# facebookresearch/generative-recommenders

Measured on NVIDIA H100. Metric: user-seqs/sec HSTU-large L=8192 d=256 bf16 fwd+bwd, higher is better.
Workload: dtype bf16

## Files before the change

generative_recommenders_b200/csrc/attn_wgmma_bwd.cu:

```cuda
#include "attn_wgmma_bwd.cuh"

namespace hstu {

template <int D, bool BF16>
__global__ void __launch_bounds__(kAttnThreads, 1) attn_bwd_wgmma_kernel(const __grid_constant__ BwdParams p) {
  bwd_key_tile<D, D, BF16, true>(p);
}

template <int D, bool BF16>
__global__ void __launch_bounds__(kAttnThreads, split_min_blocks(D)) attn_bwd_dkdv_wgmma_kernel(const __grid_constant__ BwdParams p) {
  bwd_key_tile<D, D, BF16, false>(p);
}

template <int D, bool BF16>
__global__ void __launch_bounds__(kAttnThreads, split_min_blocks(D)) attn_bwd_dq_wgmma_kernel(const __grid_constant__ BwdParams p) {
  bwd_dq_body<D, D, BF16>(p);
}

template <bool BF16>
__global__ void dq_convert_kernel(const float* __restrict__ acc, uint16_t* __restrict__ dq, long long rows, int heads, int D,
                                  long long row_stride, long long head_stride, float scale) {
  const long long nvec = rows * heads * (D / 8);
  for (long long idx = (long long)blockIdx.x * blockDim.x + threadIdx.x; idx < nvec; idx += (long long)gridDim.x * blockDim.x) {
    const int v = (int)(idx % (D / 8));
// ... 33 lines not shown
static bool split_dq(const hstu_attn_params& p) {
  return p.dqk == 32 || p.dqk == 256 || p.dqk != p.dv || p.deterministic != 0;
}

static bool fp16_copies(const hstu_attn_params& p) { return p.dtype == HSTU_BF16 && p.dqk == 32 && p.dv == 32; }

size_t wgmma_workspace_bytes(const hstu_attn_params& p, bool bwd) {
  if (!bwd && p.delta_q_len > 0) return wgmma_delta_workspace_bytes(p);
  if (fp16_copies(p)) return fp16_operands_workspace_bytes(p, bwd);
  if (!bwd || split_dq(p)) return 0;
  return (size_t)p.total_rows * p.heads * p.dqk * sizeof(float);
}

template <int D, bool BF16, bool kSplit>
static int launch_bwd_wgmma(const hstu_attn_params& p, cudaStream_t st, const Fp16Operands* f16 = nullptr) {
  if constexpr (kSplit) {
    return launch_bwd_split<D, D, BF16>(p, st, attn_bwd_dkdv_wgmma_kernel<D, BF16>, attn_bwd_dq_wgmma_kernel<D, BF16>, f16);
  } else {
    using Cfg = BwdCfg<D, D, true>;
    const size_t need = wgmma_workspace_bytes(p, true);
    if (p.workspace == nullptr || p.workspace_bytes < need) {
      set_error("hstu_attn_bwd: workspace of %zu bytes required (got %zu)", need, p.workspace_bytes);
      return HSTU_ERR_WORKSPACE;
    }
    const BwdOperands o = bwd_operands(p, f16);
    BwdParams bp = bwd_params(p, f16);
    if (int e = make_tmap_rows_heads(&bp.tmQ, o.src[0], p.total_rows, p.heads, D, o.rs[0], o.hs[0], Cfg::BOX_COLS, Cfg::BQ)) return e;
    if (int e = make_tmap_rows_heads(&bp.tmK, o.src[1], p.total_rows, p.heads, D, o.rs[1], o.hs[1], Cfg::BOX_COLS, Cfg::BKV)) return e;
    if (int e = make_tmap_rows_heads(&bp.tmV, o.src[2], p.total_rows, p.heads, D, o.rs[2], o.hs[2], Cfg::BOX_COLS, Cfg::BKV)) return e;
    if (int e = make_tmap_rows_heads(&bp.tmDO, o.src[3], p.total_rows, p.heads, D, o.rs[3], o.hs[3], Cfg::BOX_COLS, Cfg::BQ)) return e;
    HSTU_CUDA_OK(cudaMemsetAsync(p.workspace, 0, need, st));
    auto kern = attn_bwd_wgmma_kernel<D, BF16>;
    HSTU_CUDA_OK(cudaFuncSetAttribute(kern, cudaFuncAttributeMaxDynamicSharedMemorySize, Cfg::SMEM_BYTES));
    dim3 grid((p.max_seq_len + Cfg::BKV - 1) / Cfg::BKV, p.heads, p.batch);
    kern<<<grid, kAttnThreads, Cfg::SMEM_BYTES, st>>>(bp);
    HSTU_CUDA_OK(cudaGetLastError());
    const long long nvec = p.total_rows * p.heads * (D / 8);
    long long blocks = (nvec + 255) / 256;
    if (blocks > 132 * 16) blocks = 132 * 16;
    dq_convert_kernel<BF16><<<(int)blocks, 256, 0, st>>>(bp.dq_acc, reinterpret_cast<uint16_t*>(p.dq), p.total_rows, p.heads, D,
                                                         p.dq_row_stride, p.dq_head_stride, bp.dk_scale);
    HSTU_CUDA_OK(cudaGetLastError());
    return 0;
  }
}

int attn_wgmma_bwd(const hstu_attn_params& p, cudaStream_t st) {
  if (p.dqk != p.dv) return attn_wgmma_bwd_mixed(p, st);
  const bool bf = p.dtype == HSTU_BF16;
  const bool split = split_dq(p);
  switch (p.dqk) {
    case 32: {
      if (!bf) return launch_bwd_wgmma<32, false, true>(p, st);
      Fp16Operands f16;
      if (int e = fp16_operands_prepass(p, true, &f16, st)) return e;
      return launch_bwd_wgmma<32, false, true>(p, st, &f16);
    }
    case 64:
      if (split) return bf ? launch_bwd_wgmma<64, true, true>(p, st) : launch_bwd_wgmma<64, false, true>(p, st);
      return bf ? launch_bwd_wgmma<64, true, false>(p, st) : launch_bwd_wgmma<64, false, false>(p, st);
    case 128:
      if (split) return bf ? launch_bwd_wgmma<128, true, true>(p, st) : launch_bwd_wgmma<128, false, true>(p, st);
      return bf ? launch_bwd_wgmma<128, true, false>(p, st) : launch_bwd_wgmma<128, false, false>(p, st);
    case 256:
      return bf ? launch_bwd_wgmma<256, true, true>(p, st) : launch_bwd_wgmma<256, false, true>(p, st);
  }
  set_error("wgmma backward: unsupported head dim %d", p.dqk);
// ... 5 lines not shown
```

generative_recommenders_b200/csrc/attn_wgmma_bwd.cuh:

```cuda
#pragma once
#include <string.h>

#include <type_traits>

#include "attn_fp16_operands.cuh"
#include "attn_wgmma_qtile.cuh"
#include "common.cuh"
#include "internal.h"
#include "wgmma.cuh"

namespace hstu {
using namespace wg;

struct alignas(64) BwdParams {
  CUtensorMap tmQ, tmK, tmV, tmDO;
  SeqArgs seq;
  void* dk;
  void* dv;
  float* dq_acc;
  void* dq;
  long long dk_row_stride, dk_head_stride, dv_row_stride, dv_head_stride, dq_row_stride, dq_head_stride;
  float dv_scale;
  float dk_scale;
  const uint32_t* amax;
// ... 34 lines not shown
  static constexpr int K_BYTES = BKV * DQK * 2, V_BYTES = BKV * DV * 2;
  static constexpr int Q_BYTES = BQ * DQK * 2, DO_BYTES = BQ * DV * 2;
  static constexpr int STAGES = DQK != DV ? 4 : DQK == 256 ? 3 : (DQK <= 32 || !FUSED_DQ) ? 4 : (DQK == 64 ? 3 : 2);
  static constexpr int DS_BYTES = BKV * BQ * 2;
  static constexpr int DQN = DQK < 64 ? DQK : 64;
  static constexpr int OFF_K = 0;
  static constexpr int OFF_V = OFF_K + K_BYTES;
  static constexpr int OFF_Q = OFF_V + V_BYTES;
  static constexpr int OFF_DO = OFF_Q + STAGES * Q_BYTES;
  static constexpr int OFF_DS = OFF_DO + STAGES * DO_BYTES;
  static constexpr int OFF_BAR = OFF_DS + (FUSED_DQ ? 4 * DS_BYTES : 0);
  static constexpr int SMEM_BYTES = OFF_BAR + 256 + 1024;
  static_assert(SMEM_BYTES * (FUSED_DQ ? 1 : split_min_blocks(DV)) <= kSmemPerSm, "shared memory budget");
  static_assert(STAGES <= 4, "BwdBars holds four stages");
};

struct BwdBars {
  uint64_t kv_full;
  uint64_t qd_full[4];
  uint32_t qd_free[4];
};

struct QTiles {
  int A, first, T;
  __device__ __forceinline__ int at(int i) const { return i < A ? i : first + (i - A); }
};

template <int DQK, int DV, bool BF16, bool FUSED_DQ>
__device__ __forceinline__ void bwd_key_tile(const BwdParams& p) {
  using Cfg = BwdCfg<DQK, DV, FUSED_DQ>;
  constexpr int SW = Cfg::SW, SWQ = Cfg::SWQ, SWV = Cfg::SWV, BQ = Cfg::BQ, NST = Cfg::STAGES;
  constexpr int NSL = Cfg::NSL, DNK = DQK / NSL, DNV = DV / NSL;
  static_assert(DNK % Cfg::BOX_COLS_Q == 0 && DNV % Cfg::BOX_COLS_V == 0, "a slice is whole boxes");
  const int b = blockIdx.z, h = blockIdx.y;
  const int n0 = (blockIdx.x / NSL) * Cfg::BKV;
  const int ck0 = (blockIdx.x % NSL) * DNK, cv0 = (blockIdx.x % NSL) * DNV;
  const long long row0 = load_index(p.seq.seq_offsets, p.seq.offsets_i64, b);
  int len = (int)(load_index(p.seq.seq_offsets, p.seq.offsets_i64, b + 1) - row0);
  if (len > p.seq.max_seq_len) {
    if (blockIdx.x == 0) {
      zero_rows(p.dk, 2, p.dk_row_stride, (long long)h * p.dk_head_stride, DQK, row0 + p.seq.max_seq_len, row0 + len);
      zero_rows(p.dv, 2, p.dv_row_stride, (long long)h * p.dv_head_stride, DV, row0 + p.seq.max_seq_len, row0 + len);
    }
    len = p.seq.max_seq_len;
  }
  if (n0 >= len) return;
  const int n_tgt = p.seq.num_targets ? (int)load_index(p.seq.num_targets, p.seq.targets_i64, b) : -1;
  const SeqMask msk = make_seq_mask(len, n_tgt, p.seq.win, p.seq.min_full, p.seq.ctx);
  const int nrows = min(Cfg::BKV, len - n0);
  QTiles qt;
  {
    int lo, hi, ctx_hi;
    q_range_for_kv_rows(msk, n0, n0 + nrows, &lo, &hi, &ctx_hi);
    qt.A = (ctx_hi + BQ - 1) / BQ;
    qt.first = max(lo / BQ, qt.A);
    qt.T = qt.A + max(0, (hi + BQ - 1) / BQ - qt.first);
  }

  uint8_t* smem = dyn_smem_1k();
  BwdBars* bars = reinterpret_cast<BwdBars*>(smem + Cfg::OFF_BAR);
  const int tid = threadIdx.x, warp = tid >> 5, lane = tid & 31;
  if (tid == 0) {
    mbar_init(&bars->kv_full, 1);
    for (int i = 0; i < NST; ++i) {
      mbar_init(&bars->qd_full[i], 1);
      bars->qd_free[i] = 0u;
    }
    fence_barrier_init();
  }
  __syncthreads();

  auto load_qd = [&](int j) {
    const int st = j % NST;
// ... 232 lines not shown
        if (kScaled) {
          k0 = scalbnf(k0, sc.e_dk), k1 = scalbnf(k1, sc.e_dk);
          v0 = scalbnf(v0, sc.e_dv), v1 = scalbnf(v1, sc.e_dv);
        }
        const bool out_bf16 = BF16 || p.amax != nullptr;
        if (has_k) *reinterpret_cast<uint32_t*>(krow + nb * 8) = out_bf16 ? pack_bf16x2(k0, k1) : pack_f16x2(k0, k1);
        *reinterpret_cast<uint32_t*>(vrow + nb * 8) = out_bf16 ? pack_bf16x2(v0, v1) : pack_f16x2(v0, v1);
      }
    }
  }
}

template <int DQK, int DV>
struct DqCfg {
  static constexpr int BM = 128;
  static constexpr int BN = DQK + DV >= 384 ? 32 : 64;
  static constexpr int SW = swizzle_bytes(DQK), SWV = swizzle_bytes(DV);
  static constexpr int BOX_COLS = SW / 2, BOX_COLS_V = SWV / 2;
  static constexpr int NBOX = DQK / BOX_COLS, NBOX_V = DV / BOX_COLS_V;
  static constexpr int Q_BOX = BM * SW, DO_BOX = BM * SWV;
  static constexpr int K_BOX = BN * SW, V_BOX = BN * SWV;
  static constexpr int Q_BYTES = BM * DQK * 2, DO_BYTES = BM * DV * 2;
  static constexpr int K_BYTES = BN * DQK * 2, V_BYTES = BN * DV * 2;
  static constexpr int STAGES = 3;
  static constexpr int OFF_Q = 0;
  static constexpr int OFF_DO = OFF_Q + Q_BYTES;
  static constexpr int OFF_K = OFF_DO + DO_BYTES;
  static constexpr int OFF_V = OFF_K + STAGES * K_BYTES;
  static constexpr int OFF_BAR = OFF_V + STAGES * V_BYTES;
  static constexpr int SMEM_BYTES = OFF_BAR + 256 + 1024;
  static_assert(SMEM_BYTES * split_min_blocks(DV) <= kSmemPerSm, "shared memory budget of split_min_blocks(dv) CTAs per SM");
};

template <int DQK, int DV, bool BF16>
__device__ __forceinline__ void bwd_dq_body(const BwdParams& p) {
  using Cfg = DqCfg<DQK, DV>;
  constexpr int SW = Cfg::SW, SWV = Cfg::SWV, BN = Cfg::BN, NST = Cfg::STAGES;
  constexpr bool kScaled = !BF16 && DQK == 32 && DV == 32;
  const int b = blockIdx.z, h = blockIdx.y;
  const int m0 = (int)(gridDim.x - 1 - blockIdx.x) * Cfg::BM;
  QTileSeq qs;
  if (!qtile_prologue<Cfg::BM, BN>(p.seq, b, h, m0, p.dq, p.dq_row_stride, p.dq_head_stride, DQK, &qs)) return;

  uint8_t* smem = dyn_smem_1k();
  KvRing<Cfg> ring{smem, &p.tmK, &p.tmV, h, qs.row0, qs.t0, qs.T};
  ring.init();
  const int tid = threadIdx.x, warp = tid >> 5, lane = tid & 31;
  if (tid == 0) {
    prefetch_tensormap(&p.tmQ);
    prefetch_tensormap(&p.tmK);
    prefetch_tensormap(&p.tmV);
    prefetch_tensormap(&p.tmDO);
    mbar_arrive_expect_tx(&ring.bars->q_full, Cfg::Q_BYTES + Cfg::DO_BYTES);
#pragma unroll
    for (int bx = 0; bx < imax(Cfg::NBOX, Cfg::NBOX_V); ++bx) {
      if (bx < Cfg::NBOX) tma_load_3d(smem + Cfg::OFF_Q + bx * Cfg::Q_BOX, &p.tmQ, &ring.bars->q_full, bx * Cfg::BOX_COLS, h, (int)(qs.row0 + m0));
      if (bx < Cfg::NBOX_V)
        tma_load_3d(smem + Cfg::OFF_DO + bx * Cfg::DO_BOX, &p.tmDO, &ring.bars->q_full, bx * Cfg::BOX_COLS_V, h, (int)(qs.row0 + m0));
    }
    ring.fill();
  }
  __syncwarp();

  const int wgi = warpgroup_index(), w = warp & 3, g = lane >> 2, t4 = lane & 3;
  const int q_base = m0 + wgi * 64 + w * 16 + g;
  const uint64_t dq0 = desc_pin(desc_kmajor<SW>(smem_u32(smem + Cfg::OFF_Q) + wgi * 64 * SW, 0));
  const uint64_t ddo0 = desc_pin(desc_kmajor<SWV>(smem_u32(smem + Cfg::OFF_DO) + wgi * 64 * SWV, 0));
  const uint64_t dk0 = desc_pin(desc_kmajor<SW>(smem_u32(smem + Cfg::OFF_K), 0));
  const uint64_t dv0 = desc_pin(desc_kmajor<SWV>(smem_u32(smem + Cfg::OFF_V), 0));
  const uint64_t dkn0 = desc_pin(desc_mnmajor<SW>(smem_u32(smem + Cfg::OFF_K), 0, Cfg::K_BOX));
  const bool fast = qs.msk.fast != 0;
  const int full_lim = full_valid_limit(qs.msk, m0);

  const BwdScales sc(p, b, h, DQK);
  float dq[DQK / 2];
// ... 54 lines not shown
    }
    wgmma_fence();
    const uint64_t kn = desc_stage(dkn0, st, Cfg::K_BYTES);
#pragma unroll
    for (int kk = 0; kk < BN / 16; ++kk) {
      wgmma_rs<DQK, BF16, 1>(dq, a_hi[kk], desc_add(kn, kk * 16 * SW), 1);
      if constexpr (BF16) wgmma_rs<DQK, BF16, 1>(dq, a_lo[kk], desc_add(kn, kk * 16 * SW), 1);
    }
    wgmma_commit();
    wgmma_wait<0>();
    fence_regs(dq);
    fence_regs(a_hi);
    fence_regs(a_lo);
    ring.release(kKey, i, st);
    __syncwarp();
    cur.advance();
  };
  for (int i = 0; i < qs.T - 1; ++i) tile(i, std::false_type{});
  tile(qs.T - 1, std::true_type{});

#pragma unroll
  for (int hh = 0; hh < 2; ++hh) {
    const int qi = q_base + hh * 8;
    if (qi - m0 < qs.mrows) {
      uint16_t* qrow = reinterpret_cast<uint16_t*>(p.dq) + (qs.row0 + qi) * p.dq_row_stride + (long long)h * p.dq_head_stride;
#pragma unroll
      for (int nb = 0; nb < DQK / 8; ++nb) {
        float a = dq[nb * 4 + hh * 2] * p.dk_scale, c = dq[nb * 4 + hh * 2 + 1] * p.dk_scale;
        if (kScaled) a = scalbnf(a, sc.e_dq), c = scalbnf(c, sc.e_dq);
        *reinterpret_cast<uint32_t*>(qrow + nb * 8 + 2 * t4) = (BF16 || p.amax != nullptr) ? pack_bf16x2(a, c) : pack_f16x2(a, c);
      }
    }
  }
}


struct BwdOperands {
  const void* src[4];
  long long rs[4], hs[4];
};
inline BwdOperands bwd_operands(const hstu_attn_params& p, const Fp16Operands* f16) {
  BwdOperands o = {{p.q, p.k, p.v, p.dout},
                   {p.q_row_stride, p.k_row_stride, p.v_row_stride, p.do_row_stride},
                   {p.q_head_stride, p.k_head_stride, p.v_head_stride, p.do_head_stride}};
  if (f16)
    for (int i = 0; i < 4; ++i) o.src[i] = f16->copy[i], o.rs[i] = (long long)p.heads * p.dqk, o.hs[i] = p.dqk;
  return o;
}
inline BwdParams bwd_params(const hstu_attn_params& p, const Fp16Operands* f16) {
  BwdParams bp;
  memset(&bp, 0, sizeof(bp));
  if (f16) bp.amax = f16->amax;
  bp.seq = seq_args(p);
  bp.dk = p.dk;
  bp.dv = p.dv_out;
  bp.dq_acc = reinterpret_cast<float*>(p.workspace);
  bp.dq = p.dq;
  bp.dk_row_stride = p.dk_row_stride;
  bp.dk_head_stride = p.dk_head_stride;
  bp.dv_row_stride = p.dv_row_stride;
  bp.dv_head_stride = p.dv_head_stride;
  bp.dq_row_stride = p.dq_row_stride;
  bp.dq_head_stride = p.dq_head_stride;
  bp.dv_scale = 1.0f / (float)p.max_seq_len;
  bp.dk_scale = 0.5f * p.alpha / (float)p.max_seq_len;
  return bp;
}

template <int DQK, int DV, bool BF16>
int launch_bwd_split(const hstu_attn_params& p, cudaStream_t st, void (*kdkdv)(BwdParams), void (*kdq)(BwdParams),
                     const Fp16Operands* f16 = nullptr) {
  using Cfg = BwdCfg<DQK, DV, false>;
  const BwdOperands o = bwd_operands(p, f16);
  const int d[4] = {DQK, DQK, DV, DV};
  BwdParams bp = bwd_params(p, f16);
  if (int e = make_tmap_rows_heads(&bp.tmQ, o.src[0], p.total_rows, p.heads, d[0], o.rs[0], o.hs[0], Cfg::BOX_COLS_Q, Cfg::BQ)) return e;
  if (int e = make_tmap_rows_heads(&bp.tmK, o.src[1], p.total_rows, p.heads, d[1], o.rs[1], o.hs[1], Cfg::BOX_COLS, Cfg::BKV)) return e;
  if (int e = make_tmap_rows_heads(&bp.tmV, o.src[2], p.total_rows, p.heads, d[2], o.rs[2], o.hs[2], Cfg::BOX_COLS_V, Cfg::BKV)) return e;
  if (int e = make_tmap_rows_heads(&bp.tmDO, o.src[3], p.total_rows, p.heads, d[3], o.rs[3], o.hs[3], Cfg::BOX_COLS_V, Cfg::BQ)) return e;
  HSTU_CUDA_OK(cudaFuncSetAttribute(kdkdv, cudaFuncAttributeMaxDynamicSharedMemorySize, Cfg::SMEM_BYTES));
  const int key_ctas = (p.max_seq_len + Cfg::BKV - 1) / Cfg::BKV * Cfg::NSL;
  kdkdv<<<dim3(key_ctas, p.heads, p.batch), kAttnThreads, Cfg::SMEM_BYTES, st>>>(bp);
  HSTU_CUDA_OK(cudaGetLastError());
  using QC = DqCfg<DQK, DV>;
  if (int e = make_tmap_rows_heads(&bp.tmQ, o.src[0], p.total_rows, p.heads, d[0], o.rs[0], o.hs[0], QC::BOX_COLS, QC::BM)) return e;
  if (int e = make_tmap_rows_heads(&bp.tmK, o.src[1], p.total_rows, p.heads, d[1], o.rs[1], o.hs[1], QC::BOX_COLS, QC::BN)) return e;
  if (int e = make_tmap_rows_heads(&bp.tmV, o.src[2], p.total_rows, p.heads, d[2], o.rs[2], o.hs[2], QC::BOX_COLS_V, QC::BN)) return e;
  if (int e = make_tmap_rows_heads(&bp.tmDO, o.src[3], p.total_rows, p.heads, d[3], o.rs[3], o.hs[3], QC::BOX_COLS_V, QC::BM)) return e;
  HSTU_CUDA_OK(cudaFuncSetAttribute(kdq, cudaFuncAttributeMaxDynamicSharedMemorySize, QC::SMEM_BYTES));
  kdq<<<dim3((p.max_seq_len + QC::BM - 1) / QC::BM, p.heads, p.batch), kAttnThreads, QC::SMEM_BYTES, st>>>(bp);
  HSTU_CUDA_OK(cudaGetLastError());
  return 0;
}

}
```

generative_recommenders_b200/csrc/attn_wgmma_fwd.cuh:

```cuda
#pragma once
#include <string.h>

#include <algorithm>
#include <type_traits>

#include "attn_fp16_operands.cuh"
#include "attn_wgmma_qtile.cuh"
#include "common.cuh"
#include "internal.h"
#include "wgmma.cuh"

namespace hstu {
using namespace wg;

struct alignas(64) FwdParams {
  CUtensorMap tmQ, tmK, tmV;
  SeqArgs seq;
  void* out;
  long long o_row_stride, o_head_stride;
  float inv_n;
  const uint32_t* amax;
  int delta;
  float* part;
};
// ... 6 lines not shown
  static constexpr int BOX_COLS = SW / 2;
  static constexpr int BOX_COLS_V = SWV / 2;
  static constexpr int Q_BOX = BM * SW;
  static constexpr int K_BOX = BN * SW;
  static constexpr int V_BOX = BN * SWV;
  static constexpr int Q_BYTES = BM * DQK * 2;
  static constexpr int K_BYTES = BN * DQK * 2;
  static constexpr int V_BYTES = BN * DV * 2;
  static constexpr int NBOX = DQK / BOX_COLS;
  static constexpr int NBOX_V = DV / BOX_COLS_V;
  static constexpr int STAGES = (DQK == 256) ? 2 : 3;
  static constexpr int OFF_Q = 0;
  static constexpr int OFF_K = OFF_Q + Q_BYTES;
  static constexpr int OFF_V = OFF_K + STAGES * K_BYTES;
  static constexpr int OFF_BAR = OFF_V + STAGES * V_BYTES;
  static constexpr int SMEM_BYTES = OFF_BAR + 256 + 1024;
  static_assert(SMEM_BYTES <= 232448, "shared memory budget");
  static_assert(DQK <= DV, "dqk > dv has no instantiation");
};
template <int DV> constexpr int kFwdMinBlocks = (DV <= 64) ? 2 : 1;

struct DeltaRows {
  long long out_row, part_row;
  int rows;
};
template <int BM>
__device__ __forceinline__ DeltaRows delta_rows(const FwdParams& p) {
  const int m0 = (int)blockIdx.y * BM;
  const long long r = (long long)(blockIdx.x / p.seq.heads) * p.delta + m0;
  return {r, (long long)blockIdx.z * (gridDim.x / p.seq.heads) * p.delta + r, min(BM, p.delta - m0)};
}

template <int DQK, int DV, bool BF16, bool kDelta>
__device__ __forceinline__ void attn_fwd_wgmma_body(const FwdParams& p) {
  using Cfg = FwdCfg<DQK, DV>;
  constexpr int SW = Cfg::SW, SWV = Cfg::SWV, BN = Cfg::BN, NST = Cfg::STAGES;
  constexpr bool kMerge = DV <= 64;
  const int b = kDelta ? (int)blockIdx.x / p.seq.heads : (int)blockIdx.z, h = kDelta ? (int)blockIdx.x % p.seq.heads : (int)blockIdx.y;
  const int m0 = kDelta ? (int)blockIdx.y * Cfg::BM : (int)(gridDim.x - 1 - blockIdx.x) * Cfg::BM;
  QTileSeq qs;
  if constexpr (kDelta) {
    seq_rows(p.seq, b, &qs);
  } else if (!qtile_rows(p.seq, b, h, m0, p.out, p.o_row_stride, p.o_head_stride, DV, &qs)) {
    return;
  }
  const int p0 = kDelta ? qs.len - p.delta + m0 : m0;
  key_tiles<Cfg::BM, BN>(p.seq, b, p0, (kDelta ? p.delta : qs.len) - m0, &qs);
  if constexpr (kDelta) {
    const int per = (qs.T + (int)gridDim.z - 1) / (int)gridDim.z;
    qs.t0 += (int)blockIdx.z * per;
    qs.T = min(per, qs.T - (int)blockIdx.z * per);
    if (qs.T <= 0) {
      const DeltaRows dr = delta_rows<Cfg::BM>(p);
      for (int idx = threadIdx.x; idx < dr.rows * DV; idx += kAttnThreads) {
        if (gridDim.z > 1) p.part[((dr.part_row + idx / DV) * p.seq.heads + h) * DV + idx % DV] = 0.f;
        else reinterpret_cast<uint16_t*>(p.out)[(dr.out_row + idx / DV) * p.o_row_stride + (long long)h * p.o_head_stride + idx % DV] = 0;
      }
      return;
    }
  }

  uint8_t* smem = dyn_smem_1k();
  KvRing<Cfg> ring{smem, &p.tmK, &p.tmV, h, qs.row0, qs.t0, qs.T};
  ring.init();
  const int tid = threadIdx.x, warp = tid >> 5, lane = tid & 31;
  if (tid == 0) {
    prefetch_tensormap(&p.tmQ);
    prefetch_tensormap(&p.tmK);
    prefetch_tensormap(&p.tmV);
    mbar_arrive_expect_tx(&ring.bars->q_full, Cfg::Q_BYTES);
#pragma unroll
    for (int bx = 0; bx < Cfg::NBOX; ++bx)
      tma_load_3d(smem + Cfg::OFF_Q + bx * Cfg::Q_BOX, &p.tmQ, &ring.bars->q_full, bx * Cfg::BOX_COLS, h,
                  kDelta ? b * p.delta + m0 : (int)(qs.row0 + m0));
    ring.fill();
  }
  __syncwarp();

  const int wgi = kDelta ? warp >> 2 : warpgroup_index(), w = warp & 3, g = lane >> 2, t4 = lane & 3;
  if constexpr (kDelta) {
    if (wgi * 64 >= qs.mrows) {
      ring.wait(kKey, 0, 0);
      ring.release(kKey, 0, 0);
      for (int i = 0; i < qs.T; ++i) {
        const int st = i % NST;
        const bool next = i + 1 < qs.T;
        const int n0 = (qs.t0 + i) * BN;
        ring.wait(kVal, st, (i / NST) & 1);
        if (n0 + BN > qs.len) zero_tile_rows_sync<BN, SWV, Cfg::NBOX_V, kAttnThreads>(smem + Cfg::OFF_V + st * Cfg::V_BYTES, qs.len - n0);
        if (next) ring.wait(kKey, (i + 1) % NST, ((i + 1) / NST) & 1);
        __syncwarp();
        ring.release(kVal, i, st);
        if (next) ring.release(kKey, i + 1, (i + 1) % NST);
        __syncwarp();
      }
      return;
    }
  }
  const int q_base = p0 + wgi * 64 + w * 16 + g;
  const bool rows_idle = kDelta && wgi * 64 + w * 16 >= qs.mrows;
  const uint64_t dq0 = desc_pin(desc_kmajor<SW>(smem_u32(smem + Cfg::OFF_Q) + wgi * 64 * SW, 0));
  const uint64_t dk0 = desc_pin(desc_kmajor<SW>(smem_u32(smem + Cfg::OFF_K), 0));
  const uint64_t dv0 = desc_pin(desc_mnmajor<SWV>(smem_u32(smem + Cfg::OFF_V), 0, Cfg::V_BOX));
  const bool fast = qs.msk.fast != 0;
  const int full_lim = full_valid_limit(qs.msk, p0);
  constexpr bool kScaled = !kDelta && !BF16 && DQK == 32 && DV == 32;
  float c_s = p.seq.alpha_half, c_p = 1.f;
  int e_out = 0;
  if (kScaled && p.amax != nullptr) {
    const OperandExps ex = operand_exps(p.amax + ((long long)b * p.seq.heads + h) * kAmaxSlots, 2.f * p.seq.alpha_half, DQK);
    c_s = ldexpf(p.seq.alpha_half, -(ex.q + ex.k));
    c_p = pow2f(ex.p);
    e_out = -(ex.p + ex.v);
  }

  float o[DV / 2];
#pragma unroll
  for (int e = 0; e < DV / 2; ++e) o[e] = 0.f;
  uint32_t a_hi[BN / 16][4], a_lo[BN / 16][4];
#pragma unroll
  for (int kk = 0; kk < BN / 16; ++kk)
#pragma unroll
    for (int r = 0; r < 4; ++r) a_hi[kk][r] = a_lo[kk][r] = 0u;
  float s[BN / 2];
  auto issue_s = [&](int st) {
    const uint64_t kd = desc_stage(dk0, st, Cfg::K_BYTES);
#pragma unroll
    for (int ks = 0; ks < DQK / 16; ++ks) {
      const int kb = ks * 32, bx = kb / SW, off = kb % SW;
      wgmma_ss<BN, BF16, 0, 0>(s, desc_add(dq0, bx * Cfg::Q_BOX + off), desc_add(kd, bx * Cfg::K_BOX + off), ks > 0);
    }
  };
  mbar_wait(&ring.bars->q_full, 0);
  ring.wait(kKey, 0, 0);
  wgmma_fence();
  issue_s(0);
  wgmma_commit();
  wgmma_wait<0>();
  fence_regs(s);
// ... 101 lines not shown
int launch_fwd_wgmma(const hstu_attn_params& p, cudaStream_t st, void (*kern)(FwdParams), const Fp16Operands* f16 = nullptr) {
  using Cfg = FwdCfg<DQK, DV>;
  FwdParams fp;
  memset(&fp, 0, sizeof(fp));
  const int chunks = kDelta ? delta_chunks(p) : 1;
  if (chunks > 1) {
    const size_t need = wgmma_delta_workspace_bytes(p);
    if (p.workspace == nullptr || p.workspace_bytes < need) {
      set_error("hstu_attn_fwd: delta_q workspace of %zu bytes required (got %zu)", need, p.workspace_bytes);
      return HSTU_ERR_WORKSPACE;
    }
    fp.part = reinterpret_cast<float*>(p.workspace);
  }
  const long long q_rows = kDelta ? (long long)p.batch * p.delta_q_len : p.total_rows;
  if (f16) {
    const long long crs = (long long)p.heads * DQK, chs = DQK;
    if (int e = make_tmap_rows_heads(&fp.tmQ, f16->copy[0], p.total_rows, p.heads, DQK, crs, chs, Cfg::BOX_COLS, Cfg::BM)) return e;
    if (int e = make_tmap_rows_heads(&fp.tmK, f16->copy[1], p.total_rows, p.heads, DQK, crs, chs, Cfg::BOX_COLS, Cfg::BN)) return e;
    if (int e = make_tmap_rows_heads(&fp.tmV, f16->copy[2], p.total_rows, p.heads, DV, crs, chs, Cfg::BOX_COLS_V, Cfg::BN)) return e;
    fp.amax = f16->amax;
  } else {
    if (int e = make_tmap_rows_heads(&fp.tmQ, p.q, q_rows, p.heads, DQK, p.q_row_stride, p.q_head_stride, Cfg::BOX_COLS, Cfg::BM)) return e;
    if (int e = make_tmap_rows_heads(&fp.tmK, p.k, p.total_rows, p.heads, DQK, p.k_row_stride, p.k_head_stride, Cfg::BOX_COLS, Cfg::BN)) return e;
    if (int e = make_tmap_rows_heads(&fp.tmV, p.v, p.total_rows, p.heads, DV, p.v_row_stride, p.v_head_stride, Cfg::BOX_COLS_V, Cfg::BN)) return e;
  }
  fp.seq = seq_args(p);
  fp.out = p.out;
  fp.o_row_stride = p.o_row_stride;
  fp.o_head_stride = p.o_head_stride;
  fp.inv_n = 1.0f / (float)p.max_seq_len;
  fp.delta = p.delta_q_len;
  HSTU_CUDA_OK(cudaFuncSetAttribute(kern, cudaFuncAttributeMaxDynamicSharedMemorySize, Cfg::SMEM_BYTES));
  const dim3 grid = kDelta ? dim3(p.batch * p.heads, (p.delta_q_len + Cfg::BM - 1) / Cfg::BM, chunks)
                           : dim3((p.max_seq_len + Cfg::BM - 1) / Cfg::BM, p.heads, p.batch);
  kern<<<grid, kAttnThreads, Cfg::SMEM_BYTES, st>>>(fp);
  HSTU_CUDA_OK(cudaGetLastError());
  if (chunks > 1) return launch_delta_reduce(BF16, fp.part, p.out, q_rows, p.heads, DV, chunks, p.o_row_stride, p.o_head_stride, fp.inv_n, st);
  return 0;
}

}
```

generative_recommenders_b200/csrc/attn_wgmma_fwd_e4m3.cu:

```cuda
#include <string.h>

#include "attn_fp16_operands.cuh"
#include "common.cuh"
#include "internal.h"
#include "wgmma.cuh"

namespace hstu {
using namespace wg;

struct alignas(64) E4m3FwdParams {
  CUtensorMap tmQ, tmK, tmV;
  const void* seq_offsets;
  const void* num_targets;
  void* out;
  long long o_row_stride, o_head_stride;
  const float* descale[3];
  long long ds_batch[3], ds_head[3];
  int offsets_i64, targets_i64;
  int max_seq_len;
  int win, min_full, ctx;
  float alpha_half;
  float alpha;
  float inv_n;
};

template <int D>
struct E4m3FwdCfg {
  static constexpr int BM = 128;
  static constexpr int BN = 64;
  static constexpr int SWK = D >= 128 ? 128 : D;
  static constexpr int SWV = 2 * D >= 128 ? 128 : 2 * D;
  static constexpr int QK_BOX_COLS = SWK, V_BOX_COLS = SWV / 2;
  static constexpr int NBOX_QK = D / QK_BOX_COLS, NBOX_V = D / V_BOX_COLS;
  static constexpr int Q_BOX = BM * SWK, K_BOX = BN * SWK, V_BOX = BN * SWV;
  static constexpr int Q_BYTES = BM * D, K_BYTES = BN * D, V_BYTES = BN * D * 2;
  static constexpr int STAGES = 3;
  static constexpr int OFF_Q = 0;
  static constexpr int OFF_K = OFF_Q + Q_BYTES;
  static constexpr int OFF_V = OFF_K + STAGES * K_BYTES;
  static constexpr int OFF_BAR = OFF_V + STAGES * V_BYTES;
  static constexpr int SMEM_BYTES = OFF_BAR + 256 + 1024;
  static_assert(SMEM_BYTES <= 232448, "shared memory budget");
  static_assert(OFF_K % 1024 == 0 && OFF_V % 1024 == 0 && K_BYTES % 256 == 0 && V_BYTES % 1024 == 0, "swizzle atom alignment");
};
constexpr int kE4m3Threads = 256;
template <int D> constexpr int kE4m3MinBlocks = (D <= 64) ? 2 : 1;

struct E4m3Bars {
  uint64_t q_full;
  uint64_t k_full[3], v_full[3];
  uint32_t k_free[3], v_free[3];
};

__device__ __forceinline__ float load_descale(const float* d, long long bs, long long hs, int b, int h) {
  return d ? d[(long long)b * bs + (long long)h * hs] : 1.f;
}

template <int D>
__global__ void __launch_bounds__(kE4m3Threads, kE4m3MinBlocks<D>) attn_fwd_e4m3_wgmma_kernel(const __grid_constant__ E4m3FwdParams p) {
  using Cfg = E4m3FwdCfg<D>;
  constexpr int SWK = Cfg::SWK, SWV = Cfg::SWV, BN = Cfg::BN, NST = Cfg::STAGES;
  constexpr bool kMerge = D <= 64;
  const int b = blockIdx.z, h = blockIdx.y;
  const int m0 = (int)(gridDim.x - 1 - blockIdx.x) * Cfg::BM;
  const long long row0 = load_index(p.seq_offsets, p.offsets_i64, b);
  int len = (int)(load_index(p.seq_offsets, p.offsets_i64, b + 1) - row0);
  if (len > p.max_seq_len) {
    if (blockIdx.x == 0) zero_rows(p.out, 2, p.o_row_stride, (long long)h * p.o_head_stride, D, row0 + p.max_seq_len, row0 + len);
    len = p.max_seq_len;
  }
  if (m0 >= len) return;
  const int n_tgt = p.num_targets ? (int)load_index(p.num_targets, p.targets_i64, b) : -1;
  const SeqMask msk = make_seq_mask(len, n_tgt, p.win, p.min_full, p.ctx);
  const int mrows = min(Cfg::BM, len - m0);
  int lo, hi;
  kv_range_for_q_rows(msk, m0, m0 + mrows, &lo, &hi);
  const int t0 = lo / BN;
  const int T = (hi + BN - 1) / BN - t0;

  extern __shared__ uint8_t smem_raw[];
  uint8_t* smem = reinterpret_cast<uint8_t*>((reinterpret_cast<uintptr_t>(smem_raw) + 1023) & ~uintptr_t(1023));
  E4m3Bars* bars = reinterpret_cast<E4m3Bars*>(smem + Cfg::OFF_BAR);
  const int tid = threadIdx.x, warp = tid >> 5, lane = tid & 31;
  if (tid == 0) {
    mbar_init(&bars->q_full, 1);
    for (int i = 0; i < NST; ++i) {
      mbar_init(&bars->k_full[i], 1);
      mbar_init(&bars->v_full[i], 1);
      bars->k_free[i] = bars->v_free[i] = 0u;
    }
    fence_barrier_init();
  }
  __syncthreads();

  const int key_row0 = (int)(row0 + (long long)t0 * BN);
  auto load_k = [&](int i) {
    const int st = i % NST;
    mbar_arrive_expect_tx(&bars->k_full[st], Cfg::K_BYTES);
#pragma unroll
    for (int bx = 0; bx < Cfg::NBOX_QK; ++bx)
      tma_load_3d(smem + Cfg::OFF_K + st * Cfg::K_BYTES + bx * Cfg::K_BOX, &p.tmK, &bars->k_full[st], bx * Cfg::QK_BOX_COLS, h,
                  key_row0 + i * BN);
  };
  auto load_v = [&](int i) {
// ... 176 lines not shown
  return 0;
}

template <int D>
static int launch_fwd_e4m3(const hstu_attn_params& p, const hstu_attn_descales& ds, const void* v16, cudaStream_t st) {
  using Cfg = E4m3FwdCfg<D>;
  E4m3FwdParams fp;
  memset(&fp, 0, sizeof(fp));
  if (int e = make_tmap_rows_heads(&fp.tmQ, p.q, p.total_rows, p.heads, D, p.q_row_stride, p.q_head_stride, Cfg::QK_BOX_COLS, Cfg::BM, 1))
    return e;
  if (int e = make_tmap_rows_heads(&fp.tmK, p.k, p.total_rows, p.heads, D, p.k_row_stride, p.k_head_stride, Cfg::QK_BOX_COLS, Cfg::BN, 1))
    return e;
  if (int e = make_tmap_rows_heads(&fp.tmV, v16, p.total_rows, p.heads, D, (long long)p.heads * D, D, Cfg::V_BOX_COLS, Cfg::BN, 2))
    return e;
  fp.seq_offsets = p.seq_offsets;
  fp.num_targets = p.num_targets;
  fp.out = p.out;
  fp.o_row_stride = p.o_row_stride;
  fp.o_head_stride = p.o_head_stride;
  fp.descale[0] = ds.q, fp.ds_batch[0] = ds.q_batch_stride, fp.ds_head[0] = ds.q_head_stride;
  fp.descale[1] = ds.k, fp.ds_batch[1] = ds.k_batch_stride, fp.ds_head[1] = ds.k_head_stride;
  fp.descale[2] = ds.v, fp.ds_batch[2] = ds.v_batch_stride, fp.ds_head[2] = ds.v_head_stride;
  fp.offsets_i64 = p.offsets_are_i64;
  fp.targets_i64 = p.num_targets_are_i64;
  fp.max_seq_len = p.max_seq_len;
  fp.win = p.max_attn_len;
  fp.min_full = p.min_full_attn_seq_len;
  fp.ctx = p.contextual_seq_len;
  fp.alpha_half = 0.5f * p.alpha;
  fp.alpha = p.alpha;
  fp.inv_n = 1.0f / (float)p.max_seq_len;
  auto kern = attn_fwd_e4m3_wgmma_kernel<D>;
  HSTU_CUDA_OK(cudaFuncSetAttribute(kern, cudaFuncAttributeMaxDynamicSharedMemorySize, Cfg::SMEM_BYTES));
  dim3 grid((p.max_seq_len + Cfg::BM - 1) / Cfg::BM, p.heads, p.batch);
  kern<<<grid, kE4m3Threads, Cfg::SMEM_BYTES, st>>>(fp);
  HSTU_CUDA_OK(cudaGetLastError());
  return 0;
}

int attn_wgmma_fwd_e4m3(const hstu_attn_params& p, const hstu_attn_descales& ds, cudaStream_t st) {
  if (int e = e4m3_fwd_check(p)) return e;
  const void* v16 = nullptr;
  if (int e = e4m3_v_prepass(p, &v16, st)) return e;
  switch (p.dqk) {
    case 32: return launch_fwd_e4m3<32>(p, ds, v16, st);
    case 64: return launch_fwd_e4m3<64>(p, ds, v16, st);
    case 128: return launch_fwd_e4m3<128>(p, ds, v16, st);
    case 256: return launch_fwd_e4m3<256>(p, ds, v16, st);
  }
  set_error("fp8 attention: unsupported head dim %d", p.dqk);
  return HSTU_ERR_UNSUPPORTED;
}

}
```

generative_recommenders_b200/csrc/attn_wgmma_qtile.cuh:

```cuda
#pragma once
#include <type_traits>

#include "common.cuh"
#include "internal.h"
#include "wgmma.cuh"

namespace hstu {
using namespace wg;

constexpr int kAttnThreads = 256;

struct SeqArgs {
  const void* seq_offsets;
  const void* num_targets;
  int offsets_i64, targets_i64;
  int max_seq_len, heads;
  int win, min_full, ctx;
  float alpha_half;
};
inline SeqArgs seq_args(const hstu_attn_params& p) {
  return {p.seq_offsets,  p.num_targets,           p.offsets_are_i64,    p.num_targets_are_i64, p.max_seq_len, p.heads,
          p.max_attn_len, p.min_full_attn_seq_len, p.contextual_seq_len, 0.5f * p.alpha};
}

struct QTileSeq {
  long long row0;
  int len, mrows, t0, T;
  SeqMask msk;
};
__device__ __forceinline__ void seq_rows(const SeqArgs& a, int b, QTileSeq* q) {
  const long long row0 = load_index(a.seq_offsets, a.offsets_i64, b);
  q->len = (int)(load_index(a.seq_offsets, a.offsets_i64, b + 1) - row0);
  q->row0 = row0;
}
__device__ __forceinline__ bool qtile_rows(const SeqArgs& a, int b, int h, int m0, void* out, long long row_stride,
                                           long long head_stride, int d, QTileSeq* q) {
  seq_rows(a, b, q);
  if (q->len > a.max_seq_len) {
    if (blockIdx.x == 0) zero_rows(out, 2, row_stride, (long long)h * head_stride, d, q->row0 + a.max_seq_len, q->row0 + q->len);
    q->len = a.max_seq_len;
  }
  return m0 < q->len;
}

template <int BM, int BN>
__device__ __forceinline__ void key_tiles(const SeqArgs& a, int b, int p0, int rows, QTileSeq* q) {
  const int n_tgt = a.num_targets ? (int)load_index(a.num_targets, a.targets_i64, b) : -1;
  q->msk = make_seq_mask(q->len, n_tgt, a.win, a.min_full, a.ctx);
  q->mrows = min(BM, rows);
  int lo, hi;
  kv_range_for_q_rows(q->msk, p0, p0 + q->mrows, &lo, &hi);
  q->t0 = lo / BN;
  q->T = (hi + BN - 1) / BN - q->t0;
}
template <int BM, int BN>
__device__ __forceinline__ bool qtile_prologue(const SeqArgs& a, int b, int h, int m0, void* out, long long row_stride,
                                               long long head_stride, int d, QTileSeq* q) {
  if (!qtile_rows(a, b, h, m0, out, row_stride, head_stride, d, q)) return false;
  key_tiles<BM, BN>(a, b, m0, q->len - m0, q);
  return true;
}

struct QTileBars {
  uint64_t q_full;
  uint64_t k_full[3], v_full[3];
  uint32_t k_free[3], v_free[3];
};
constexpr std::false_type kKey{};
constexpr std::true_type kVal{};

template <class Cfg>
struct KvRing {
  static_assert(Cfg::STAGES <= 3, "QTileBars holds three stages");
  uint8_t* smem;
  const CUtensorMap *tmK, *tmV;
  int h;
  long long row0;
  int t0, T;
  QTileBars* bars;

  __device__ __forceinline__ void init() {
    bars = reinterpret_cast<QTileBars*>(smem + Cfg::OFF_BAR);
    if (threadIdx.x == 0) {
      mbar_init(&bars->q_full, 1);
      for (int i = 0; i < Cfg::STAGES; ++i) {
        mbar_init(&bars->k_full[i], 1);
        mbar_init(&bars->v_full[i], 1);
        bars->k_free[i] = bars->v_free[i] = 0u;
      }
      fence_barrier_init();
    }
    __syncthreads();
// ... 64 lines not shown
```

Before: 102.4.

## Reorder attention CTA grid heads-first, anchor q-tiles per sequence length, add PDL launches

Reorders the attention kernel grids so heads (times slices) run along x, tile rank along y and batch along z, so CTAs for all heads of a tile rank are scheduled together. Q-tile start rows are now counted back from each sequence's own length instead of from max_seq_len, so the heaviest causal tiles of every sequence launch first and the empty trailing CTAs land at the end. It also enables programmatic dependent launch between the dK/dV kernel and the dQ kernel in split backward, and for the fp16-operand forward. The aims are better L2 reuse of K/V across heads, less load imbalance, and overlap of kernel launch tails, at the cost of more complex launch code and grid ordering.

```diff
diff --git a/generative_recommenders_b200/csrc/attn_cta_order.cuh b/generative_recommenders_b200/csrc/attn_cta_order.cuh
--- /dev/null
+++ b/generative_recommenders_b200/csrc/attn_cta_order.cuh
@@ -0,0 +1,41 @@
+#pragma once
+#include <cuda_runtime.h>
+
+namespace hstu {
+
+struct CtaWork {
+  int rank;
+  int b, h;
+  int slice;
+};
+template <int SLICES = 1>
+__host__ __device__ __forceinline__ CtaWork cta_work(unsigned x, unsigned y, unsigned z) {
+  return {(int)y, (int)z, (int)(x / SLICES), (int)(x % SLICES)};
+}
+inline dim3 cta_grid(int ranks, int batch, int heads, int slices = 1) {
+  return dim3((unsigned)heads * (unsigned)slices, (unsigned)ranks, (unsigned)batch);
+}
+__host__ __device__ __forceinline__ int qtile_row0(int len, int bm, int rank) { return ((len + bm - 1) / bm - 1 - rank) * bm; }
+
+#ifndef HSTU_ATTN_PDL
+#define HSTU_ATTN_PDL 1
+#endif
+constexpr bool kAttnPdl = HSTU_ATTN_PDL != 0;
+__device__ __forceinline__ void grid_dep_wait() { asm volatile("griddepcontrol.wait;" ::: "memory"); }
+__device__ __forceinline__ void grid_dep_launch() { asm volatile("griddepcontrol.launch_dependents;" ::: "memory"); }
+template <class P>
+inline cudaError_t launch_attn(void (*kern)(P), dim3 grid, int smem, cudaStream_t st, bool pdl, const P& arg) {
+  cudaLaunchAttribute attr = {};
+  attr.id = cudaLaunchAttributeProgrammaticStreamSerialization;
+  attr.val.programmaticStreamSerializationAllowed = 1;
+  cudaLaunchConfig_t cfg = {};
+  cfg.gridDim = grid;
+  cfg.blockDim = dim3(256);
+  cfg.dynamicSmemBytes = (size_t)smem;
+  cfg.stream = st;
+  cfg.attrs = &attr;
+  cfg.numAttrs = pdl ? 1 : 0;
+  return cudaLaunchKernelEx(&cfg, kern, arg);
+}
+
+}
diff --git a/generative_recommenders_b200/csrc/attn_wgmma_bwd.cu b/generative_recommenders_b200/csrc/attn_wgmma_bwd.cu
--- a/generative_recommenders_b200/csrc/attn_wgmma_bwd.cu
+++ b/generative_recommenders_b200/csrc/attn_wgmma_bwd.cu
@@ -89,7 +89,7 @@
     HSTU_CUDA_OK(cudaMemsetAsync(p.workspace, 0, need, st));
     auto kern = attn_bwd_wgmma_kernel<D, BF16>;
     HSTU_CUDA_OK(cudaFuncSetAttribute(kern, cudaFuncAttributeMaxDynamicSharedMemorySize, Cfg::SMEM_BYTES));
-    dim3 grid((p.max_seq_len + Cfg::BKV - 1) / Cfg::BKV, p.heads, p.batch);
+    const dim3 grid = cta_grid((p.max_seq_len + Cfg::BKV - 1) / Cfg::BKV, p.batch, p.heads);
     kern<<<grid, kAttnThreads, Cfg::SMEM_BYTES, st>>>(bp);
     HSTU_CUDA_OK(cudaGetLastError());
     const long long nvec = p.total_rows * p.heads * (D / 8);
diff --git a/generative_recommenders_b200/csrc/attn_wgmma_bwd.cuh b/generative_recommenders_b200/csrc/attn_wgmma_bwd.cuh
--- a/generative_recommenders_b200/csrc/attn_wgmma_bwd.cuh
+++ b/generative_recommenders_b200/csrc/attn_wgmma_bwd.cuh
@@ -90,13 +90,15 @@
   constexpr int SW = Cfg::SW, SWQ = Cfg::SWQ, SWV = Cfg::SWV, BQ = Cfg::BQ, NST = Cfg::STAGES;
   constexpr int NSL = Cfg::NSL, DNK = DQK / NSL, DNV = DV / NSL;
   static_assert(DNK % Cfg::BOX_COLS_Q == 0 && DNV % Cfg::BOX_COLS_V == 0, "a slice is whole boxes");
-  const int b = blockIdx.z, h = blockIdx.y;
-  const int n0 = (blockIdx.x / NSL) * Cfg::BKV;
-  const int ck0 = (blockIdx.x % NSL) * DNK, cv0 = (blockIdx.x % NSL) * DNV;
+  if (!FUSED_DQ && kAttnPdl) grid_dep_launch();
+  const CtaWork cw = cta_work<NSL>(blockIdx.x, blockIdx.y, blockIdx.z);
+  const int b = cw.b, h = cw.h;
+  const int n0 = (int)((unsigned)cw.rank * Cfg::BKV);
+  const int ck0 = cw.slice * DNK, cv0 = cw.slice * DNV;
   const long long row0 = load_index(p.seq.seq_offsets, p.seq.offsets_i64, b);
   int len = (int)(load_index(p.seq.seq_offsets, p.seq.offsets_i64, b + 1) - row0);
   if (len > p.seq.max_seq_len) {
-    if (blockIdx.x == 0) {
+    if (cw.rank == 0 && cw.slice == 0) {
       zero_rows(p.dk, 2, p.dk_row_stride, (long long)h * p.dk_head_stride, DQK, row0 + p.seq.max_seq_len, row0 + len);
       zero_rows(p.dv, 2, p.dv_row_stride, (long long)h * p.dv_head_stride, DV, row0 + p.seq.max_seq_len, row0 + len);
     }
@@ -395,15 +397,20 @@
   static_assert(SMEM_BYTES * split_min_blocks(DV) <= kSmemPerSm, "shared memory budget of split_min_blocks(dv) CTAs per SM");
 };
 
+__device__ __forceinline__ void bwd_dq_exit() {
+  if constexpr (kAttnPdl) grid_dep_wait();
+}
+
 template <int DQK, int DV, bool BF16>
 __device__ __forceinline__ void bwd_dq_body(const BwdParams& p) {
   using Cfg = DqCfg<DQK, DV>;
   constexpr int SW = Cfg::SW, SWV = Cfg::SWV, BN = Cfg::BN, NST = Cfg::STAGES;
   constexpr bool kScaled = !BF16 && DQK == 32 && DV == 32;
-  const int b = blockIdx.z, h = blockIdx.y;
-  const int m0 = (int)(gridDim.x - 1 - blockIdx.x) * Cfg::BM;
+  const CtaWork cw = cta_work(blockIdx.x, blockIdx.y, blockIdx.z);
+  const int b = cw.b, h = cw.h;
+  int m0;
   QTileSeq qs;
-  if (!qtile_prologue<Cfg::BM, BN>(p.seq, b, h, m0, p.dq, p.dq_row_stride, p.dq_head_stride, DQK, &qs)) return;
+  if (!qtile_prologue<Cfg::BM, BN>(p.seq, cw, p.dq, p.dq_row_stride, p.dq_head_stride, DQK, &m0, &qs)) return bwd_dq_exit();
 
   uint8_t* smem = dyn_smem_1k();
   KvRing<Cfg> ring{smem, &p.tmK, &p.tmV, h, qs.row0, qs.t0, qs.T};
@@ -524,6 +531,7 @@
       }
     }
   }
+  bwd_dq_exit();
 }
 
 
@@ -571,8 +579,7 @@
   if (int e = make_tmap_rows_heads(&bp.tmV, o.src[2], p.total_rows, p.heads, d[2], o.rs[2], o.hs[2], Cfg::BOX_COLS_V, Cfg::BKV)) return e;
   if (int e = make_tmap_rows_heads(&bp.tmDO, o.src[3], p.total_rows, p.heads, d[3], o.rs[3], o.hs[3], Cfg::BOX_COLS_V, Cfg::BQ)) return e;
   HSTU_CUDA_OK(cudaFuncSetAttribute(kdkdv, cudaFuncAttributeMaxDynamicSharedMemorySize, Cfg::SMEM_BYTES));
-  const int key_ctas = (p.max_seq_len + Cfg::BKV - 1) / Cfg::BKV * Cfg::NSL;
-  kdkdv<<<dim3(key_ctas, p.heads, p.batch), kAttnThreads, Cfg::SMEM_BYTES, st>>>(bp);
+  kdkdv<<<cta_grid((p.max_seq_len + Cfg::BKV - 1) / Cfg::BKV, p.batch, p.heads, Cfg::NSL), kAttnThreads, Cfg::SMEM_BYTES, st>>>(bp);
   HSTU_CUDA_OK(cudaGetLastError());
   using QC = DqCfg<DQK, DV>;
   if (int e = make_tmap_rows_heads(&bp.tmQ, o.src[0], p.total_rows, p.heads, d[0], o.rs[0], o.hs[0], QC::BOX_COLS, QC::BM)) return e;
@@ -580,8 +587,7 @@
   if (int e = make_tmap_rows_heads(&bp.tmV, o.src[2], p.total_rows, p.heads, d[2], o.rs[2], o.hs[2], QC::BOX_COLS_V, QC::BN)) return e;
   if (int e = make_tmap_rows_heads(&bp.tmDO, o.src[3], p.total_rows, p.heads, d[3], o.rs[3], o.hs[3], QC::BOX_COLS_V, QC::BM)) return e;
   HSTU_CUDA_OK(cudaFuncSetAttribute(kdq, cudaFuncAttributeMaxDynamicSharedMemorySize, QC::SMEM_BYTES));
-  kdq<<<dim3((p.max_seq_len + QC::BM - 1) / QC::BM, p.heads, p.batch), kAttnThreads, QC::SMEM_BYTES, st>>>(bp);
-  HSTU_CUDA_OK(cudaGetLastError());
+  HSTU_CUDA_OK(launch_attn(kdq, cta_grid((p.max_seq_len + QC::BM - 1) / QC::BM, p.batch, p.heads), QC::SMEM_BYTES, st, kAttnPdl, bp));
   return 0;
 }
 
diff --git a/generative_recommenders_b200/csrc/attn_wgmma_fwd.cuh b/generative_recommenders_b200/csrc/attn_wgmma_fwd.cuh
--- a/generative_recommenders_b200/csrc/attn_wgmma_fwd.cuh
+++ b/generative_recommenders_b200/csrc/attn_wgmma_fwd.cuh
@@ -62,16 +62,21 @@
 }
 
 template <int DQK, int DV, bool BF16, bool kDelta>
+constexpr bool kScaledFwd = !kDelta && !BF16 && DQK == 32 && DV == 32;
+
+template <int DQK, int DV, bool BF16, bool kDelta>
 __device__ __forceinline__ void attn_fwd_wgmma_body(const FwdParams& p) {
   using Cfg = FwdCfg<DQK, DV>;
   constexpr int SW = Cfg::SW, SWV = Cfg::SWV, BN = Cfg::BN, NST = Cfg::STAGES;
   constexpr bool kMerge = DV <= 64;
-  const int b = kDelta ? (int)blockIdx.x / p.seq.heads : (int)blockIdx.z, h = kDelta ? (int)blockIdx.x % p.seq.heads : (int)blockIdx.y;
-  const int m0 = kDelta ? (int)blockIdx.y * Cfg::BM : (int)(gridDim.x - 1 - blockIdx.x) * Cfg::BM;
+  const CtaWork cw = kDelta ? CtaWork{(int)blockIdx.y, (int)blockIdx.x / p.seq.heads, (int)blockIdx.x % p.seq.heads, 0}
+                            : cta_work(blockIdx.x, blockIdx.y, blockIdx.z);
+  const int b = cw.b, h = cw.h;
+  int m0 = cw.rank * Cfg::BM;
   QTileSeq qs;
   if constexpr (kDelta) {
     seq_rows(p.seq, b, &qs);
-  } else if (!qtile_rows(p.seq, b, h, m0, p.out, p.o_row_stride, p.o_head_stride, DV, &qs)) {
+  } else if (!qtile_rows<Cfg::BM>(p.seq, cw, p.out, p.o_row_stride, p.o_head_stride, DV, &m0, &qs)) {
     return;
   }
   const int p0 = kDelta ? qs.len - p.delta + m0 : m0;
@@ -98,6 +103,9 @@
     prefetch_tensormap(&p.tmQ);
     prefetch_tensormap(&p.tmK);
     prefetch_tensormap(&p.tmV);
+  }
+  if constexpr (kScaledFwd<DQK, DV, BF16, kDelta>) grid_dep_wait();
+  if (tid == 0) {
     mbar_arrive_expect_tx(&ring.bars->q_full, Cfg::Q_BYTES);
 #pragma unroll
     for (int bx = 0; bx < Cfg::NBOX; ++bx)
@@ -134,7 +142,7 @@
   const uint64_t dv0 = desc_pin(desc_mnmajor<SWV>(smem_u32(smem + Cfg::OFF_V), 0, Cfg::V_BOX));
   const bool fast = qs.msk.fast != 0;
   const int full_lim = full_valid_limit(qs.msk, p0);
-  constexpr bool kScaled = !kDelta && !BF16 && DQK == 32 && DV == 32;
+  constexpr bool kScaled = kScaledFwd<DQK, DV, BF16, kDelta>;
   float c_s = p.seq.alpha_half, c_p = 1.f;
   int e_out = 0;
   if (kScaled && p.amax != nullptr) {
@@ -302,9 +310,8 @@
   fp.delta = p.delta_q_len;
   HSTU_CUDA_OK(cudaFuncSetAttribute(kern, cudaFuncAttributeMaxDynamicSharedMemorySize, Cfg::SMEM_BYTES));
   const dim3 grid = kDelta ? dim3(p.batch * p.heads, (p.delta_q_len + Cfg::BM - 1) / Cfg::BM, chunks)
-                           : dim3((p.max_seq_len + Cfg::BM - 1) / Cfg::BM, p.heads, p.batch);
-  kern<<<grid, kAttnThreads, Cfg::SMEM_BYTES, st>>>(fp);
-  HSTU_CUDA_OK(cudaGetLastError());
+                           : cta_grid((p.max_seq_len + Cfg::BM - 1) / Cfg::BM, p.batch, p.heads);
+  HSTU_CUDA_OK(launch_attn(kern, grid, Cfg::SMEM_BYTES, st, kAttnPdl && f16 != nullptr, fp));
   if (chunks > 1) return launch_delta_reduce(BF16, fp.part, p.out, q_rows, p.heads, DV, chunks, p.o_row_stride, p.o_head_stride, fp.inv_n, st);
   return 0;
 }
diff --git a/generative_recommenders_b200/csrc/attn_wgmma_fwd_e4m3.cu b/generative_recommenders_b200/csrc/attn_wgmma_fwd_e4m3.cu
--- a/generative_recommenders_b200/csrc/attn_wgmma_fwd_e4m3.cu
+++ b/generative_recommenders_b200/csrc/attn_wgmma_fwd_e4m3.cu
@@ -1,5 +1,6 @@
 #include <string.h>
 
+#include "attn_cta_order.cuh"
 #include "attn_fp16_operands.cuh"
 #include "common.cuh"
 #include "internal.h"
@@ -61,15 +62,16 @@
   using Cfg = E4m3FwdCfg<D>;
   constexpr int SWK = Cfg::SWK, SWV = Cfg::SWV, BN = Cfg::BN, NST = Cfg::STAGES;
   constexpr bool kMerge = D <= 64;
-  const int b = blockIdx.z, h = blockIdx.y;
-  const int m0 = (int)(gridDim.x - 1 - blockIdx.x) * Cfg::BM;
+  const CtaWork cw = cta_work(blockIdx.x, blockIdx.y, blockIdx.z);
+  const int b = cw.b, h = cw.h;
   const long long row0 = load_index(p.seq_offsets, p.offsets_i64, b);
   int len = (int)(load_index(p.seq_offsets, p.offsets_i64, b + 1) - row0);
   if (len > p.max_seq_len) {
-    if (blockIdx.x == 0) zero_rows(p.out, 2, p.o_row_stride, (long long)h * p.o_head_stride, D, row0 + p.max_seq_len, row0 + len);
+    if (cw.rank == 0) zero_rows(p.out, 2, p.o_row_stride, (long long)h * p.o_head_stride, D, row0 + p.max_seq_len, row0 + len);
     len = p.max_seq_len;
   }
-  if (m0 >= len) return;
+  const int m0 = qtile_row0(len, Cfg::BM, cw.rank);
+  if (m0 < 0) return;
   const int n_tgt = p.num_targets ? (int)load_index(p.num_targets, p.targets_i64, b) : -1;
   const SeqMask msk = make_seq_mask(len, n_tgt, p.win, p.min_full, p.ctx);
   const int mrows = min(Cfg::BM, len - m0);
@@ -312,7 +314,7 @@
   fp.inv_n = 1.0f / (float)p.max_seq_len;
   auto kern = attn_fwd_e4m3_wgmma_kernel<D>;
   HSTU_CUDA_OK(cudaFuncSetAttribute(kern, cudaFuncAttributeMaxDynamicSharedMemorySize, Cfg::SMEM_BYTES));
-  dim3 grid((p.max_seq_len + Cfg::BM - 1) / Cfg::BM, p.heads, p.batch);
+  const dim3 grid = cta_grid((p.max_seq_len + Cfg::BM - 1) / Cfg::BM, p.batch, p.heads);
   kern<<<grid, kE4m3Threads, Cfg::SMEM_BYTES, st>>>(fp);
   HSTU_CUDA_OK(cudaGetLastError());
   return 0;
diff --git a/generative_recommenders_b200/csrc/attn_wgmma_qtile.cuh b/generative_recommenders_b200/csrc/attn_wgmma_qtile.cuh
--- a/generative_recommenders_b200/csrc/attn_wgmma_qtile.cuh
+++ b/generative_recommenders_b200/csrc/attn_wgmma_qtile.cuh
@@ -1,6 +1,7 @@
 #pragma once
 #include <type_traits>
 
+#include "attn_cta_order.cuh"
 #include "common.cuh"
 #include "internal.h"
 #include "wgmma.cuh"
@@ -33,14 +34,16 @@
   q->len = (int)(load_index(a.seq_offsets, a.offsets_i64, b + 1) - row0);
   q->row0 = row0;
 }
-__device__ __forceinline__ bool qtile_rows(const SeqArgs& a, int b, int h, int m0, void* out, long long row_stride,
-                                           long long head_stride, int d, QTileSeq* q) {
-  seq_rows(a, b, q);
+template <int BM>
+__device__ __forceinline__ bool qtile_rows(const SeqArgs& a, const CtaWork& w, void* out, long long row_stride,
+                                           long long head_stride, int d, int* m0, QTileSeq* q) {
+  seq_rows(a, w.b, q);
   if (q->len > a.max_seq_len) {
-    if (blockIdx.x == 0) zero_rows(out, 2, row_stride, (long long)h * head_stride, d, q->row0 + a.max_seq_len, q->row0 + q->len);
+    if (w.rank == 0) zero_rows(out, 2, row_stride, (long long)w.h * head_stride, d, q->row0 + a.max_seq_len, q->row0 + q->len);
     q->len = a.max_seq_len;
   }
-  return m0 < q->len;
+  *m0 = qtile_row0(q->len, BM, w.rank);
+  return *m0 >= 0;
 }
 
 template <int BM, int BN>
@@ -54,10 +57,10 @@
   q->T = (hi + BN - 1) / BN - q->t0;
 }
 template <int BM, int BN>
-__device__ __forceinline__ bool qtile_prologue(const SeqArgs& a, int b, int h, int m0, void* out, long long row_stride,
-                                               long long head_stride, int d, QTileSeq* q) {
-  if (!qtile_rows(a, b, h, m0, out, row_stride, head_stride, d, q)) return false;
-  key_tiles<BM, BN>(a, b, m0, q->len - m0, q);
+__device__ __forceinline__ bool qtile_prologue(const SeqArgs& a, const CtaWork& w, void* out, long long row_stride,
+                                               long long head_stride, int d, int* m0, QTileSeq* q) {
+  if (!qtile_rows<BM>(a, w, out, row_stride, head_stride, d, m0, q)) return false;
+  key_tiles<BM, BN>(a, w.b, *m0, q->len - *m0, q);
   return true;
 }
 
```

After: 103.8 (median of 6 runs). +1.4%, better.
